# kofinandi/pixel-nerf-yolo

Measured on AMD Instinct MI355X. Metric: rays/sec (whole node), 64 samples/ray, 3-view 128×128 render, higher is better.
Workload: dtype f32 (matrix products on f16x2 split operands, fp32 accumulate)

## Files before the change

### pixel-nerf-yolo_amd/csrc/api.hip

```cpp
#include <algorithm>
#include <cmath>
#include <cstdio>
#include <cstdlib>
#include <cstring>
#include <map>
#include <string>
#include <vector>

#include "api_internal.h"

namespace pny {

static thread_local std::string g_err;
void set_error(const std::string& msg) { g_err = msg; }
int hip_fail(hipError_t e, const char* what) {
    g_err = std::string("HIP error: ") + hipGetErrorString(e) + " in " + what;
    return PNY_ERR_HIP;
}
int fail(int code, const std::string& msg) {
    g_err = msg;
    return code;
}

}
// ... 741 lines not shown
                           const float* focal_dev, const float* c_dev, const float* bboxes_dev,
                           const pny_train_batch_draws* draws, float* rays_dev, float* rgb_gt_dev, int32_t* pix_dev,
                           pny_stream stream) {
    const char* who = "pny_sample_train_batch: ";
    if (!d || !images_dev || !poses_dev || !focal_dev || !rays_dev || !rgb_gt_dev)
        return fail(PNY_ERR_ARG, std::string(who) + "null argument");
    if (d->n_objs < 1 || d->n_views < 1 || d->height < 1 || d->width < 1 || d->n_rays < 1)
        return fail(PNY_ERR_ARG, std::string(who) + "bad shape");
    if ((int64_t)d->n_objs * d->n_rays > INT32_MAX) return fail(PNY_ERR_ARG, std::string(who) + "more than 2^31 - 1 rays");
    if ((int64_t)d->n_views * d->height * d->width > (int64_t)UINT32_MAX)
        return fail(PNY_ERR_ARG, std::string(who) + "NV * H * W must be below 2^32");
    if ((d->focal_rows != 1 && d->focal_rows != d->n_objs) || (d->focal_cols != 1 && d->focal_cols != 2))
        return fail(PNY_ERR_ARG, std::string(who) + "focal must be (1 | SB, 1 | 2)");
    if (c_dev && d->c_rows != 1 && d->c_rows != d->n_objs) return fail(PNY_ERR_ARG, std::string(who) + "c must be (1 | SB, 2)");
    if (draws && (bboxes_dev ? (!draws->image_ids_dev || !draws->u_x_dev || !draws->u_y_dev) : !draws->pix_inds_dev))
        return fail(PNY_ERR_ARG, std::string(who) + (bboxes_dev ? "bbox mode replays image_ids_dev, u_x_dev and u_y_dev"
                                                                : "uniform mode replays pix_inds_dev"));
    if (reinterpret_cast<uintptr_t>(rays_dev) & 15) return fail(PNY_ERR_ARG, std::string(who) + "rays_dev must be 16-byte aligned");
    TrainBatchArgs a;
    a.sb = d->n_objs, a.nv = d->n_views, a.h = d->height, a.w = d->width, a.b = d->n_rays;
    a.znear = d->z_near, a.zfar = d->z_far;
    a.focal_rows = d->focal_rows, a.focal_cols = d->focal_cols, a.c_rows = c_dev ? d->c_rows : 1;
    a.seed = d->seed, a.draw_offset = draws ? 0 : d->draw_offset;
    a.images = images_dev, a.poses = poses_dev, a.focal = focal_dev, a.c = c_dev, a.bboxes = bboxes_dev;
    a.pix_inds = draws && !bboxes_dev ? draws->pix_inds_dev : nullptr;
    a.image_ids = draws && bboxes_dev ? draws->image_ids_dev : nullptr;
    a.u_x = draws && bboxes_dev ? draws->u_x_dev : nullptr;
    a.u_y = draws && bboxes_dev ? draws->u_y_dev : nullptr;
    a.rays = rays_dev, a.rgb = rgb_gt_dev, a.pix = pix_dev;
    launch_train_batch(a, (hipStream_t)stream);
    PNY_HIP(hipGetLastError());
    return PNY_OK;
}

int pny_yolo_train_batch(const pny_yolo_batch_desc* d, const float* poses_host, const int64_t* view_ids_host, const float focal[2],
                         const float c[2], const float* const* targets_dev, float* rays_dev, float* targets_out_dev,
                         int64_t* offsets_host, pny_stream stream) {
    const std::string who = "pny_yolo_train_batch: ";
    if (!d || !offsets_host) return fail(PNY_ERR_ARG, who + "null argument");
    const bool query = !rays_dev && !targets_out_dev;
    if (!query && (!poses_host || !view_ids_host || !focal || !c || !targets_dev || !rays_dev || !targets_out_dev))
        return fail(PNY_ERR_ARG, who + "null argument");
    if (d->n_scales < 1 || d->n_scales > PNY_YOLO_BATCH_MAX_SCALES) return fail(PNY_ERR_ARG, who + "n_scales must be 1 .. 4");
    if (d->n_views < 1 || d->n_views > PNY_YOLO_BATCH_MAX_VIEWS)
        return fail(PNY_ERR_ARG, who + "n_views must be 1 .. 16 (one launch carries at most 16 selected cameras)");
    if (d->n_views_all < 1 || d->height < 1 || d->width < 1) return fail(PNY_ERR_ARG, who + "bad shape");
    if (d->n_anchors < 1 || d->n_anchors > 64) return fail(PNY_ERR_ARG, who + "bad shape: n_anchors must be 1 .. 64");
    if ((reinterpret_cast<uintptr_t>(rays_dev) & 15) || (reinterpret_cast<uintptr_t>(targets_out_dev) & 3))
        return fail(PNY_ERR_ARG, who + "rays_dev must be 16-byte aligned (targets_out_dev 4-byte)");
    YoloBatchArgs a;
    memset(&a, 0, sizeof(a));
    a.n_scales = d->n_scales, a.row = d->n_anchors * 6;
    a.znear = d->z_near, a.zfar = d->z_far;
    a.rays = rays_dev, a.targets_out = targets_out_dev;
    if (!query && (focal[0] == 0.f || focal[1] == 0.f)) return fail(PNY_ERR_ARG, who + "zero focal length");
    for (int s = 0; s < d->n_scales; ++s) {
        const int cell = d->cell_sizes[s];
        if (cell < 1 || cell > d->height || cell > d->width)
            return fail(PNY_ERR_ARG, who + "every cell size must be 1 .. min(height, width)");
        a.hs[s] = d->height / cell, a.ws[s] = d->width / cell;
        a.off[s + 1] = a.off[s] + (long long)d->n_views * a.hs[s] * a.ws[s];
        if ((long long)d->n_views_all * a.hs[s] * a.ws[s] > INT32_MAX) return fail(PNY_ERR_ARG, who + "more than 2^31 - 1 cells in a grid");
        if (query) continue;
        if (!targets_dev[s] || (reinterpret_cast<uintptr_t>(targets_dev[s]) & 3)) return fail(PNY_ERR_ARG, who + "null or unaligned target grid");
        a.targets[s] = targets_dev[s];
        const float fx = focal[0] / (float)cell, fy = focal[1] / (float)cell, cx = c[0] / (float)cell, cy = c[1] / (float)cell;
        a.kinv[s][0] = (float)(1.0 / fx);
        a.kinv[s][1] = (float)(1.0 / fy);
        a.kinv[s][2] = (float)(-(double)cx / fx);
        a.kinv[s][3] = (float)(-(double)cy / fy);
    }
    if (a.off[d->n_scales] * a.row > INT32_MAX) return fail(PNY_ERR_ARG, who + "more than 2^31 - 1 target values");
    if (query) {
        for (int s = 0; s <= d->n_scales; ++s) offsets_host[s] = a.off[s];
        return PNY_OK;
    }
    for (int i = 0; i < d->n_views; ++i) {
        const int64_t v = view_ids_host[i];
        if (v < 0 || v >= d->n_views_all) return fail(PNY_ERR_ARG, who + "view id outside [0, n_views_all)");
        double inv[16];
        if (!invert4(poses_host + 16 * v, inv)) return fail(PNY_ERR_ARG, who + "singular extrinsic matrix");
        for (int r = 0; r < 3; ++r) {
            for (int q = 0; q < 3; ++q) a.pose[i][3 * r + q] = (float)inv[4 * r + q];
            a.pose[i][9 + r] = (float)inv[4 * r + 3];
        }
        a.view_id[i] = (int)v;
    }
    for (int s = 0; s <= d->n_scales; ++s) offsets_host[s] = a.off[s];
    launch_yolo_train_batch(a, (hipStream_t)stream);
    PNY_HIP(hipGetLastError());
    return PNY_OK;
}

}

namespace pny {
static unsigned range_bits(const pny_model* m) {
    return m->range_flag ? __atomic_load_n(m->range_flag, __ATOMIC_RELAXED) : 0u;
}
int check_ready(pny_scene* s, const char* who) {
    if (!s) return fail(PNY_ERR_ARG, std::string(who) + ": null scene");
    if (!s->m->finalized) return fail(PNY_ERR_STATE, std::string(who) + ": weights not finalized (pny_model_finalize)");
    const unsigned bits = s->precision == PNY_PRECISION_F32 ? 0u : range_bits(s->m);
    if (bits) {
        if (bits & PNY_RANGE_WEIGHT) s->m->f16_weights_ok = false;
        return fail(PNY_ERR_RANGE, std::string(who) + ": an earlier f16 (F16X2 / F16) launch left the f16 range (" +
                                       std::string(bits & PNY_RANGE_ACTIVATION ? "activation " : "") +
                                       std::string(bits & PNY_RANGE_GRADIENT ? "gradient " : "") +
                                       std::string(bits & PNY_RANGE_WEIGHT ? "weight " : "") +
                                       "beyond +-65504 or not finite): its results are invalid.  Clear with pny_model_range_status(m, 0, 1), pin "
                                       "pny_scene_set_precision(s, PNY_PRECISION_F32) and repeat the call");
    }
    if (!s->have_latent) return fail(PNY_ERR_STATE, std::string(who) + ": scene has no latent (pny_scene_encode / pny_scene_set_latent)");
    if (!s->have_cams) return fail(PNY_ERR_STATE, std::string(who) + ": scene has no cameras (pny_scene_set_cameras)");
    if (s->cam_ns != s->ns) return fail(PNY_ERR_STATE, std::string(who) + ": camera count != latent view count");
    if (s->n_objs > 1 && s->ns % s->n_objs)
        return fail(PNY_ERR_STATE, std::string(who) + ": grouped scene: the view count is not a multiple of the object count");
    if (obj_views(s) > 1 && s->m->desc.combine_layer >= s->m->desc.n_blocks)
        return fail(PNY_ERR_ARG, std::string(who) + ": multi-view scene needs combine_layer < n_blocks");
    return 0;
}

int view_blocks(const pny_model_desc& d) { return d.combine_layer < d.n_blocks ? d.combine_layer : d.n_blocks; }
}

namespace pny {
double mlp_flops_per_point(const pny_model_desc& d, int ns, MlpPass pass) {
    const int nvb = view_blocks(d);
    const double per_view = (pass == PASS_CHAIN ? 0.0 : (double)d_in(d) * HID) +
                            (pass == PASS_FORWARD ? (double)nvb * d.d_latent * HID : 0.0) + 2.0 * nvb * HID * HID;
    const double post = 2.0 * (d.n_blocks - nvb) * HID * HID + (double)HID * d.d_out;
    const double once = pass == PASS_FORWARD_VIEW_MEAN ? (double)(ns - 1) * HID * HID : 0.0;
    return 2.0 * (ns * per_view + post - once);
}
}

enum MlpKernel { K_F32_8x64 = MLP_8x64, K_F32_16x64 = MLP_16x64, K_F32_8x32 = MLP_8x32, K_H2, K_H2S, K_H1 };
struct MlpRoute {
    MlpKernel kernel;
    Prec prec;
    bool stash;
    bool projected;
    int tile;
    int grid_cap;
};

static bool f16_default(const pny_scene* s) {
    const pny_model* m = s->m;
    return s->precision != PNY_PRECISION_F32 && m->f16_weights_ok && mlp_h2_supports(m->desc.n_blocks, m->desc.combine_layer);
}

static bool wants_projection(const pny_scene* s, long long n_points, bool force) {
    if (!s->m->has_zproj) return false;
    if ((long long)s->hl * s->wl * view_blocks(s->m->desc) * HID >= (1ll << 31)) return false;
    if (force) return true;
    if (s->zp_mode == PNY_PROJECTION_OFF) return false;
    return s->zp_mode != PNY_PROJECTION_AUTO || f16_default(s) || n_points >= 2ll * s->hl * s->wl;
}

static MlpRoute route_mlp(const pny_scene* s, long long n_points, bool stash) {
    const pny_model_desc& d = s->m->desc;
    const int prec = s->precision;
    const bool can_f16 = prec != PNY_PRECISION_F32 && (s->m->f16_weights_ok || prec == PNY_PRECISION_F16X2) &&
                         mlp_h2_supports(d.n_blocks, d.combine_layer) && (!stash || s->L % 128 == 0);
    MlpRoute r;
    r.stash = stash;
    r.projected = stash ? can_f16 && wants_projection(s, n_points, true) : wants_projection(s, n_points, false);
    const bool f16 = r.projected && can_f16;
    const bool h1 = f16 && (prec == PNY_PRECISION_F16_TRAIN || (prec == PNY_PRECISION_F16 && !stash));
    bool h2s = f16 && !h1 && !stash && n_points <= 32ll * mlp_max_grid(MLP_8x64);
    if (f16 && !h1 && !stash)
        if (const char* e = getenv("PNYOLO_H2_SPLIT")) h2s = atoi(e) != 0;
    const int shape = (f16 || stash) ? MLP_8x64 : mlp_pick_variant(n_points);
    r.kernel = h1 ? K_H1 : h2s ? K_H2S : f16 ? K_H2 : MlpKernel(shape);
    r.prec = h1 ? PREC_H1 : f16 ? PREC_H2 : PREC_F32;
    r.tile = h2s ? 32 : mlp_tile_samples(shape);
    r.grid_cap = h2s ? 2 * mlp_max_grid(MLP_8x64) : mlp_max_grid(shape);
    if (!stash)
        if (const char* e = getenv("PNYOLO_GRID")) {
            const int g = atoi(e);
            if (g > 0 && g < r.grid_cap) r.grid_cap = g;
        }
    return r;
}

namespace pny {
static int project_latent(const pny_scene* s, int which, float* out, hipStream_t st, int* route) {
    const pny_model* m = s->m;
    if (!m->desc.has_fine) which = 0;
    const long long npix = (long long)s->ns * s->hl * s->wl;
    if (!run_pixel_linear(m->zproj[which], s->latent.f(), npix, out, st, f16_default(s), route))
        return fail(PNY_ERR_HIP, "latent projection launch failed");
    return 0;
}

int ensure_projection(pny_scene* s, int which, long long n_points, hipStream_t st, const float** zp, bool force) {
    *zp = nullptr;
    const pny_model* m = s->m;
    if (!wants_projection(s, n_points, force)) return 0;
    const int nvb = view_blocks(m->desc);
    if (s->zp_generation != m->generation) {
        s->zp_valid[0] = s->zp_valid[1] = false;
        s->zp_generation = m->generation;
    }
    if (!m->desc.has_fine) which = 0;
    if (!s->zp_valid[which]) {
        const long long npix = (long long)s->ns * s->hl * s->wl;
        int rc;
        if ((rc = s->zp[which].reserve((size_t)npix * nvb * HID * sizeof(float)))) return rc;
        if ((rc = project_latent(s, which, s->zp[which].f(), st, nullptr))) return rc;
        s->zp_valid[which] = true;
    }
    *zp = s->zp[which].f();
    return 0;
}
}

namespace pny {
int fill_mlp_args(pny_scene* s, int mode, const float* xyz, const float* dirs, const float* rays, const float* z, int K,
                  long long n_points, int coarse, float* out, MlpArgs* pa) {
    const pny_model_desc& d = s->m->desc;
    MlpArgs& a = *pa;
    memset(&a, 0, sizeof(a));
    const bool fine_w = !(coarse || !d.has_fine || !s->m->use_fine);
    a.w = fine_w ? s->m->fine : s->m->coarse;
    a.n_blocks = d.n_blocks;
    use_images(a, f16_images(s->m, fine_w, false));
    a.range_flag = s->m->range_flag;
    a.latent = s->latent.f();
    a.zp = nullptr;
    a.zp_stride = view_blocks(d) * HID;
    a.tap_stride = s->L;
    memcpy(a.cams, s->cams, sizeof(Cam) * (size_t)s->ns);
    a.xyz = xyz;
    a.dirs = dirs;
    a.rays = rays;
    a.z = z;
    a.out = out;
    a.n_points = n_points;
    a.K = K;
    a.mode = mode;
    a.NS = obj_views(s);
    a.obj_pts = 0;
    if (s->n_objs > 1) {
        if (n_points % s->n_objs || (n_points / s->n_objs) % 64)
            return fail(PNY_ERR_ARG, "grouped scene: every object's share of the samples must be the same multiple of 64");
        a.obj_pts = n_points / s->n_objs;
    }
    a.L = s->L;
    a.Hl = s->hl;
    a.Wl = s->wl;
    a.combine_layer = d.combine_layer;
    a.d_out = d.d_out;
    a.yolo = d.yolo;
    a.num_freqs = d.num_freqs;
    a.freq_factor = d.freq_factor;
    const float lsx = (float)s->wl / ((float)s->wl - 1.0f) * 2.0f;
    const float lsy = (float)s->hl / ((float)s->hl - 1.0f) * 2.0f;
    a.sx = lsx / (float)s->width;
    a.sy = lsy / (float)s->height;
    const long long tiles = (n_points + 63) / 64;
    if (tiles > 0x7fffffffll) return fail(PNY_ERR_ARG, "too many points for one launch");
    a.n_tiles = (int)tiles;
    a.idx32 = (tiles * 64) < 0xffffffffll;
    if (mode == 1 && (reinterpret_cast<uintptr_t>(rays) & 15)) return fail(PNY_ERR_ARG, "rays must be 16-byte aligned");
    int rc;
    if ((rc = s->scratch.reserve(mlp_scratch_floats() * sizeof(float)))) return rc;
    a.scratch = s->scratch.f();
    return 0;
}
}

static int run_mlp(pny_scene* s, int mode, const float* xyz, const float* dirs, const float* rays, const float* z,
                   int K, long long n_points, int coarse, float* out, hipStream_t st, int stash_pass = -1) {
    if (n_points == 0) return 0;
    pny_model* m = s->m;
    const pny_model_desc& d = m->desc;
    MlpArgs a;
    int rc;
    if ((rc = fill_mlp_args(s, mode, xyz, dirs, rays, z, K, n_points, coarse, out, &a))) return rc;
    const bool fine_w = !(coarse || !d.has_fine || !m->use_fine);
    const int which = fine_w ? 1 : 0;
    bool room = false;
    if (stash_pass >= 0) {
        s->stashed[stash_pass].valid = false;
        room = m->defer && obj_views(s) == m->defer_ns && m->defer_used[which] + a.n_tiles <= m->defer_cap[which];
    }
    const MlpRoute r = route_mlp(s, n_points, room);
    if (r.stash) {
        pny_scene::StashedPass& sp = s->stashed[stash_pass];
        a.lay = stash_layout(d, obj_views(s), s->L);
        a.stash_x = a.lay.x_record(m->dx_stash[which].f(), m->defer_used[which]);
        sp.valid = true;
        sp.epoch = m->defer_epoch;
        sp.which = which;
        sp.tile0 = m->defer_used[which];
        sp.tiles = a.n_tiles;
        sp.n_points = n_points;
        m->defer_used[which] += a.n_tiles;
    }
    if (r.projected) {
        if ((rc = ensure_projection(s, which, n_points, st, &a.zp, r.stash))) return rc;
        a.tap_stride = a.zp_stride;
    }
    if (r.kernel == K_H1) {
        if ((rc = want_h1_images(m, s->precision == PNY_PRECISION_F16_TRAIN))) return rc;
        use_images(a, f16_images(m, fine_w, true));
// ... 274 lines not shown
```

### pixel-nerf-yolo_amd/csrc/mlp_h2.hip

```cpp
#include <cstdlib>
#include <cstring>
#include <cstdio>
#include <vector>

#include "mlp_bwd_core.h"
#include "mlp_h2_core.h"

#if PNY_H2_PLANES == 1
#define PNY_H2_KERNEL pny_mlp_h1_kernel
#elif defined(PNY_H2_SPLIT)
#define PNY_H2_KERNEL pny_mlp_h2s_kernel
#else
#define PNY_H2_KERNEL pny_mlp_h2_kernel
#endif

namespace pny {

#ifdef PNY_H2_STAMP
enum { HS_TOTAL = 0, HS_GEMM, HS_GATHER_WAIT, HS_GATHER, HS_EPI_WAIT, HS_EPI, HS_PROLOGUE, HS_LINOUT, HS_SLAB, HS_REAL, HS_N };
__device__ unsigned long long* g_h2_stamp_buf;
__device__ __forceinline__ unsigned long long h2now() {
    unsigned long long t;
    __builtin_amdgcn_sched_barrier(0);
    asm volatile("s_memtime %0\n\ts_waitcnt lgkmcnt(0)" : "=s"(t)::"memory");
// ... 57 lines not shown
            }
            __builtin_amdgcn_sched_barrier(0);
#pragma unroll
            for (int q = 0; q < 4; ++q) {
                char* s0 = base + (4 * nt + q) * (2 * ROW_BYTES) + 32 * mt * 16;
                float x0 = acc[nt][mt][4 * q + 0] + b[q].x, x1 = acc[nt][mt][4 * q + 1] + b[q].y;
                float x2 = acc[nt][mt][4 * q + 2] + b[q].z, x3 = acc[nt][mt][4 * q + 3] + b[q].w;
                if (ADDZ) {
                    x0 += za[q].x;
                    x1 += za[q].y;
                    x2 += zb[q].x;
                    x3 += zb[q].y;
                }
                acc[nt][mt][4 * q + 0] = x0;
                acc[nt][mt][4 * q + 1] = x1;
                acc[nt][mt][4 * q + 2] = x2;
                acc[nt][mt][4 * q + 3] = x3;
                const float r0 = relu1(x0), r1 = relu1(x1), r2 = relu1(x2), r3 = relu1(x3);
                if constexpr (STASH) stash_store(stash, stash_lane, stash_off + (unsigned)(((8 * nt + 2 * q) * TM + 32 * mt) * 16), r0, r1, r2, r3);
                h2put_planes(s0, r0, r1, r2, r3, rmax);
            }
        }
    }
    range_check(rmax, range_flag);
}

struct SlabRef {
    __amdgpu_buffer_rsrc_t rsrc;
    unsigned lane_off;
};
__device__ __forceinline__ void h2slab_store(const f32x16 (&h)[h2::NT][h2::MT], const SlabRef& sl) {
    using namespace h2;
#pragma unroll
    for (int nt = 0; nt < NT; ++nt)
#pragma unroll
        for (int mt = 0; mt < MT; ++mt)
#pragma unroll
            for (int q = 0; q < 4; ++q) {
                const f32x4 v = {h[nt][mt][4 * q + 0], h[nt][mt][4 * q + 1], h[nt][mt][4 * q + 2], h[nt][mt][4 * q + 3]};
                __builtin_amdgcn_raw_buffer_store_b128(__builtin_bit_cast(u32x4, v), sl.rsrc,
                                                       sl.lane_off + (unsigned)(((nt * MT + mt) * 4 + q) * 64 * 16), 0, 2);
            }
}
__device__ __forceinline__ void h2slab_load(f32x16 (&t)[h2::NT][h2::MT], const SlabRef& sl) {
    using namespace h2;
#pragma unroll
    for (int nt = 0; nt < NT; ++nt)
#pragma unroll
        for (int mt = 0; mt < MT; ++mt)
#pragma unroll
            for (int q = 0; q < 4; ++q) {
                const u32x4 u = __builtin_amdgcn_raw_buffer_load_b128(sl.rsrc, sl.lane_off, (unsigned)(((nt * MT + mt) * 4 + q) * 64 * 16), 2);
                const f32x4 v = __builtin_bit_cast(f32x4, u);
                t[nt][mt][4 * q + 0] = v.x;
                t[nt][mt][4 * q + 1] = v.y;
                t[nt][mt][4 * q + 2] = v.z;
                t[nt][mt][4 * q + 3] = v.w;
            }
}

#ifndef PNY_H2_SLAB_DEPTH
#define PNY_H2_SLAB_DEPTH 4
#endif
struct SlabPipe {
    static constexpr int SD = PNY_H2_SLAB_DEPTH;
    static_assert(SD >= 2, "slab pipeline");
    f32x4 buf[SD][4];
};
__device__ __forceinline__ void h2slab_issue(SlabPipe& sp, int p, const SlabRef& sh, const SlabRef& sr) {
    const SlabRef& s = (p & 1) ? sh : sr;
#pragma unroll
    for (int q = 0; q < 4; ++q)
        sp.buf[p % SlabPipe::SD][q] =
            __builtin_bit_cast(f32x4, __builtin_amdgcn_raw_buffer_load_b128(s.rsrc, s.lane_off, (unsigned)(((p >> 1) * 4 + q) * 64 * 16), 2));
}
__device__ __forceinline__ void h2view_sum(f32x16 (&net)[h2::NT][h2::MT], f32x16 (&h)[h2::NT][h2::MT], const float* bias, const SlabRef& sh,
                                           const SlabRef& sr, bool add, bool store, int wave, int lane) {
    using namespace h2;
    SlabPipe sp;
    const float* bl = bias + 32 * NT * wave + 4 * (lane >> 5);
    constexpr int NP = 2 * NT * MT, SD = SlabPipe::SD;
    if (add) {
#pragma unroll
        for (int p = 0; p + 1 < SD; ++p) h2slab_issue(sp, p, sh, sr);
    }
#pragma unroll
    for (int p = 0; p < NP; ++p) {
        const int nt = (p >> 1) / MT, mt = (p >> 1) % MT;
        if (add) {
            if (p + SD - 1 < NP) h2slab_issue(sp, p + SD - 1, sh, sr);
            __builtin_amdgcn_sched_barrier(0);
        }
        f32x16& t = (p & 1) ? h[nt][mt] : net[nt][mt];
#pragma unroll
        for (int q = 0; q < 4; ++q) {
            if (!(p & 1)) {
                const float4 b = *reinterpret_cast<const float4*>(bl + 32 * nt + 8 * q);
                t[4 * q + 0] = relu1(t[4 * q + 0] + b.x);
                t[4 * q + 1] = relu1(t[4 * q + 1] + b.y);
                t[4 * q + 2] = relu1(t[4 * q + 2] + b.z);
                t[4 * q + 3] = relu1(t[4 * q + 3] + b.w);
            }
            if (add) {
#pragma unroll
                for (int i = 0; i < 4; ++i) t[4 * q + i] = t[4 * q + i] + sp.buf[p % SD][q][i];
            }
            if (store) {
                const SlabRef& s = (p & 1) ? sh : sr;
                const f32x4 v = {t[4 * q + 0], t[4 * q + 1], t[4 * q + 2], t[4 * q + 3]};
                __builtin_amdgcn_raw_buffer_store_b128(__builtin_bit_cast(u32x4, v), s.rsrc, s.lane_off + (unsigned)(((p >> 1) * 4 + q) * 64 * 16), 0, 2);
            }
        }
        if (add) __builtin_amdgcn_sched_barrier(0);
    }
}

__device__ __forceinline__ void h2mean_planes(const f32x16 (&net)[h2::NT][h2::MT], f32x16 (&h)[h2::NT][h2::MT], float rns, char* planes, int wave,
                                              int lane, unsigned* range_flag) {
    using namespace h2;
    float rmax = 0.f;
    char* base = planes + (4 * NT * wave) * (2 * ROW_BYTES) + (lane & 31) * 16 + 8 * (lane >> 5);
#pragma unroll
    for (int nt = 0; nt < NT; ++nt)
#pragma unroll
        for (int mt = 0; mt < MT; ++mt)
#pragma unroll
            for (int q = 0; q < 4; ++q) {
                char* s0 = base + (4 * nt + q) * (2 * ROW_BYTES) + 32 * mt * 16;
                const float r0 = net[nt][mt][4 * q + 0] * rns, r1 = net[nt][mt][4 * q + 1] * rns;
                const float r2 = net[nt][mt][4 * q + 2] * rns, r3 = net[nt][mt][4 * q + 3] * rns;
                h2put_planes(s0, r0, r1, r2, r3, rmax);
#pragma unroll
                for (int i = 0; i < 4; ++i) h[nt][mt][4 * q + i] = h[nt][mt][4 * q + i] * rns;
            }
    range_check(rmax, range_flag);
}

template <int B>
__device__ __forceinline__ void h2gather_commit(const GatherTaps<h2::C, 2>& g, char* planes, int chunk, int wave, int lane) {
    using namespace h2;
    constexpr int NMB = GatherTaps<C>::NMB, QSTEP = GatherTaps<C>::QSTEP;
    const int m = (wave % NMB) * 8 + (lane & 7);
    char* base = planes + (16 * chunk + (lane >> 4)) * (2 * ROW_BYTES) + m * 16 + 8 * ((lane >> 3) & 1);
#pragma unroll
    for (int i = 0; i < GatherTaps<C>::QPW; ++i) {
        const int qb = wave / NMB + i * QSTEP;
        const float4 r = tap_blend(g.x[B][i], g.w);
        char* s0 = base + (4 * qb) * (2 * ROW_BYTES);
        *reinterpret_cast<float2*>(s0) = make_float2(r.x, r.y);
        *reinterpret_cast<float2*>(s0 + ROW_BYTES) = make_float2(r.z, r.w);
    }
}

template <bool STASH>
__device__ __forceinline__ void h2prologue(const MlpArgs& a, int v, long long tile, char* planes, float4* tap_tab, int tid, unsigned* range_flag,
                                           __amdgpu_buffer_rsrc_t stash = __amdgpu_buffer_rsrc_t(), unsigned stash_xin = 0, float4* tap_raw = nullptr) {
    using namespace h2;
    constexpr int NPART = THREADS / TM;
    const int m = tid % TM, part = tid / TM;
    long long s = tile * TM + m;
    if (s >= a.n_points) s = a.n_points - 1;
    float p[3], d[3];
    load_point(a, s, p, d);
    const Cam cam = a.cams[tile_view_base(a, tile * TM) + v];
    float xr[3], xc[3], vd[3];
    camera_point(cam, p, d, xr, xc, vd);
    float rmax = 0.f;
    for (int g = part; g < D_IN_PAD / 4; g += NPART) {
        const float e0 = input_entry(4 * g + 0, xr, vd, a.freq_factor, a.num_freqs), e1 = input_entry(4 * g + 1, xr, vd, a.freq_factor, a.num_freqs);
        const float e2 = input_entry(4 * g + 2, xr, vd, a.freq_factor, a.num_freqs), e3 = input_entry(4 * g + 3, xr, vd, a.freq_factor, a.num_freqs);
        if constexpr (STASH) stash_store(stash, (unsigned)((g * TM + m) * 16), stash_xin, e0, e1, e2, e3);
        h2put_planes<true>(planes + (g >> 1) * (2 * ROW_BYTES) + m * 16 + 8 * (g & 1), e0, e1, e2, e3, rmax);
    }
    range_check(rmax, range_flag);
    if (part == NPART - 1) {
        int pix[4], offs[4];
        float wgt[4];
        pixel_taps(a, cam, xc, 1, pix, wgt);
#pragma unroll
        for (int k = 0; k < 4; ++k) offs[k] = pix[k] * a.tap_stride;
        tap_record(tap_tab, m, offs, wgt);
        if constexpr (STASH) {
#pragma unroll
            for (int k = 0; k < 4; ++k) offs[k] = pix[k] * a.L;
            tap_record(tap_raw, m, offs, wgt);
        }
    }
}

template <bool STASH>
__global__ __launch_bounds__(h2::THREADS, 2) void PNY_H2_KERNEL(const MlpArgs a) {
    using namespace h2;
    extern __shared__ __attribute__((aligned(16))) char smem_raw[];
    char* planes = smem_raw;
    float4* tap_tab = reinterpret_cast<float4*>(smem_raw + ACT_BYTES);
    float* bias_tab = reinterpret_cast<float*>(smem_raw + ACT_BYTES + TAP_BYTES);
    float4* tap_raw = reinterpret_cast<float4*>(smem_raw + lds_bytes(a.n_blocks));
    const int tid = threadIdx.x, lane = tid & 63, wave = __builtin_amdgcn_readfirstlane(tid >> 6);
    const SlabRef slab = {__builtin_amdgcn_make_buffer_rsrc(a.scratch + (size_t)blockIdx.x * (TM * HID), 0, TM * HID * 4, 0x00020000),
                          (unsigned)((wave * (NT * MT * 16 * 64) + 4 * lane) * 4)};
#if defined(PNY_H2_PER_VIEW_FC1) || PNY_H2_PLANES == 1
    constexpr bool VIEW_MEAN = false;
#else
    constexpr bool VIEW_MEAN = !STASH;
#endif
    const SlabRef slab_r = {__builtin_amdgcn_make_buffer_rsrc(a.scratch + ((size_t)gridDim.x + blockIdx.x) * (TM * HID), 0, TM * HID * 4, 0x00020000),
                            slab.lane_off};
    const int nb = a.n_blocks;
    const int nvb = a.combine_layer < nb ? a.combine_layer : nb;
    const WStream ws = wstream(a, lane);
    const H2Seg s_in = h2seg(ws, a.h2_in, D_IN_PAD / 16, wave);
    auto fc0seg = [&](int b) { return h2seg(ws, a.h2_fc0[b], HID / 16, wave); };
    auto fc1seg = [&](int b) { return h2seg(ws, a.h2_fc1[b], HID / 16, wave); };
    auto entry_bias = [&](int b) -> const float* {
        if constexpr (LDS_BIAS) return bias_tab + (b == 0 ? 0 : 2 * b) * HID;
        return b == 0 ? a.w.b_in : a.w.b_fc1[b - 1];
    };
    auto fc0_bias = [&](int b) -> const float* {
        if constexpr (LDS_BIAS) return bias_tab + (1 + 2 * b) * HID;
        return a.w.b_fc0[b];
    };
    H2Ring ring;
    h2ring_fill(ring, ws, s_in);
#ifdef PNY_H2_STAMP
    unsigned long long hs_acc[HS_N], hs_t_ = 0;
    for (int i = 0; i < HS_N; ++i) hs_acc[i] = 0;
    const unsigned long long hs_start = h2now();
    const unsigned long long hs_real0 = __builtin_amdgcn_s_memrealtime();
#endif
    if constexpr (LDS_BIAS) {
        for (int i = tid; i < (1 + 2 * nb) * HID; i += THREADS) {
            const int vec = i / HID, f = i % HID;
            const float* src = vec == 0 ? a.w.b_in : ((vec & 1) ? a.w.b_fc0[(vec - 1) >> 1] : a.w.b_fc1[(vec - 2) >> 1]);
            bias_tab[i] = src[f];
        }
    }

    const TileWalk tw = tile_walk(a.n_tiles);
    for (long long tile = tw.first; tile < tw.last; tile += tw.step) {
        f32x16 h[NT][MT];
        f32x16 net[NT][MT];
        GatherTaps<C, 2> g;
        __amdgpu_buffer_rsrc_t xr = __amdgpu_buffer_rsrc_t();
        if constexpr (STASH)
            xr = stash_rsrc(a.lay.x_record(a.stash_x, tile), a.lay.x_tile);
        auto block_tail = [&](int blk, const H2Seg& after, bool slab_in, int next_c0, unsigned stash_net) {
            HS_T0();
            h2zero<NT, MT>(net);
            __syncthreads();
            HS_LAP(HS_EPI_WAIT);
            h2gemm(net, ring, ws, fc0seg(blk), fc1seg(blk), planes, lane);
            HS_LAP(HS_GEMM);
            __syncthreads();
            HS_LAP(HS_EPI_WAIT);
            h2epilogue<false, STASH>(net, fc0_bias(blk), planes, wave, lane, a.range_flag, xr, stash_net);
            if (!VIEW_MEAN && slab_in) {
                h2slab_load(net, slab);
                HS_LAP(HS_EPI);
                __syncthreads();
                HS_LAP(HS_EPI_WAIT);
                h2gemm(h, ring, ws, fc1seg(blk), after, planes, lane);
                HS_LAP(HS_GEMM);
#pragma unroll
                for (int nt = 0; nt < NT; ++nt)
#pragma unroll
                    for (int mt = 0; mt < MT; ++mt)
#pragma unroll
                        for (int r = 0; r < 16; ++r) h[nt][mt][r] = net[nt][mt][r] + h[nt][mt][r];
            } else if (next_c0 >= 0) {
                HS_LAP(HS_EPI);
                __syncthreads();
                HS_LAP(HS_EPI_WAIT);
                h2gemm(h, ring, ws, fc1seg(blk), after, planes, lane, [&]() { gather_issue<C, 0>(g, next_c0, wave); });
                HS_LAP(HS_GEMM);
            } else {
                HS_LAP(HS_EPI);
                __syncthreads();
                HS_LAP(HS_EPI_WAIT);
                h2gemm(h, ring, ws, fc1seg(blk), after, planes, lane);
                HS_LAP(HS_GEMM);
            }
        };
        for (int v = 0; v < a.NS; ++v) {
            const int vb = tile_view_base(a, tile * TM);
            const H2Seg after_view = v + 1 < a.NS ? s_in : (nvb < nb ? fc0seg(nvb) : s_in);
            const unsigned x_view = STASH ? stash_bytes((unsigned)v * (unsigned)a.lay.x_view) : 0u;
            auto act_slot = [&](int i) { return x_view + stash_bytes((unsigned)a.lay.o_act + (unsigned)i * (unsigned)STASH_SLOT); };
            HS_T0();
            __syncthreads();
            h2prologue<STASH>(a, v, tile, planes, tap_tab, tid, a.range_flag, xr, x_view + stash_bytes((unsigned)a.lay.o_in), tap_raw);
            h2zero<NT, MT>(h);
            __syncthreads();
            if constexpr (STASH) {
                const unsigned xz = x_view + stash_bytes((unsigned)a.lay.o_z);
                gather_setup<C>(g, a.latent + (size_t)(vb + v) * a.Hl * a.Wl * a.L, tap_raw, wave, lane);
                const int nch = a.L / GCH;
                const unsigned zlane = (unsigned)(((lane >> 3) * TM + (wave % 8) * 8 + (lane & 7)) * 16);
                auto put = [&](const float4(&x)[4][4], int c) {
#pragma unroll
                    for (int i = 0; i < 4; ++i) {
                        const float4 r = tap_blend(x[i], g.w);
                        stash_store(xr, zlane, xz + (unsigned)((32 * c + 8 * i) * TM * 16), r.x, r.y, r.z, r.w);
                    }
                };
                gather_issue<C, 0>(g, 0, wave);
                for (int c = 0; c < nch; c += 2) {
                    if (c + 1 < nch) gather_issue<C, 1>(g, (c + 1) * GCH, wave);
                    __builtin_amdgcn_sched_barrier(0);
                    put(g.x[0], c);
                    if (c + 2 < nch) gather_issue<C, 0>(g, (c + 2) * GCH, wave);
                    __builtin_amdgcn_sched_barrier(0);
                    if (c + 1 < nch) put(g.x[1], c + 1);
                }
            }
            gather_setup<C>(g, a.zp + (size_t)(vb + v) * a.Hl * a.Wl * a.zp_stride, tap_tab, wave, lane);
            gather_issue<C, 0>(g, 0, wave);
            HS_LAP(HS_PROLOGUE);
            h2gemm(h, ring, ws, s_in, fc0seg(0), planes, lane);
            HS_LAP(HS_GEMM);
            auto block_entry = [&](int blk) {
                const int cb = blk * HID;
                HS_LAP(HS_GATHER);
                __syncthreads();
                HS_LAP(HS_GATHER_WAIT);
                gather_issue<C, 1>(g, cb + GCH, wave);
                __builtin_amdgcn_sched_barrier(0);
                h2gather_commit<0>(g, planes, 0, wave, lane);
                gather_issue<C, 0>(g, cb + 2 * GCH, wave);
                __builtin_amdgcn_sched_barrier(0);
                h2gather_commit<1>(g, planes, 1, wave, lane);
                gather_issue<C, 1>(g, cb + 3 * GCH, wave);
                __builtin_amdgcn_sched_barrier(0);
                h2gather_commit<0>(g, planes, 2, wave, lane);
                h2gather_commit<1>(g, planes, 3, wave, lane);
                HS_LAP(HS_GATHER);
                __syncthreads();
                HS_LAP(HS_GATHER_WAIT);
                h2epilogue<true, STASH>(h, entry_bias(blk), planes, wave, lane, a.range_flag, xr, act_slot(2 * blk));
                HS_LAP(HS_EPI);
            };
            auto view_block = [&](int blk, const H2Seg& after, bool slab_in, int next_c0) {
                block_entry(blk);
                block_tail(blk, after, slab_in, next_c0, act_slot(2 * blk + 1));
            };
            auto mean_tail = [&](int blk) {
                const bool last = v + 1 == a.NS;
                HS_T0();
                h2zero<NT, MT>(net);
                __syncthreads();
                HS_LAP(HS_EPI_WAIT);
                h2gemm(net, ring, ws, fc0seg(blk), last ? fc1seg(blk) : s_in, planes, lane);
                HS_LAP(HS_GEMM);
                h2view_sum(net, h, fc0_bias(blk), slab, slab_r, v > 0, !last, wave, lane);
                if (!last) {
                    HS_LAP(HS_SLAB);
                    return;
                }
                HS_LAP(v > 0 ? HS_SLAB : HS_EPI);
                __syncthreads();
                HS_LAP(HS_EPI_WAIT);
                h2mean_planes(net, h, 1.0f / (float)a.NS, planes, wave, lane, a.range_flag);
                HS_LAP(HS_EPI);
                __syncthreads();
                HS_LAP(HS_EPI_WAIT);
                h2gemm(h, ring, ws, fc1seg(blk), after_view, planes, lane);
                HS_LAP(HS_GEMM);
            };
#if defined(PNY_H2_NOPREFETCH)
            for (int blk = 0; blk + 1 < nvb; ++blk) {
                view_block(blk, fc0seg(blk + 1), false, -1);
                gather_issue<C, 0>(g, (blk + 1) * HID, wave);
            }
#else
            for (int blk = 0; blk + 1 < nvb; ++blk) view_block(blk, fc0seg(blk + 1), false, (blk + 1) * HID);
#endif
            if constexpr (VIEW_MEAN) {
                block_entry(nvb - 1);
                mean_tail(nvb - 1);
            } else {
                view_block(nvb - 1, after_view, v > 0, -1);
            }
            if (!VIEW_MEAN && a.NS > 1) {
                HS_T0();
                if (v + 1 < a.NS) {
                    h2slab_store(h, slab);
                } else {
                    const float rns = 1.0f / (float)a.NS;
#pragma unroll
                    for (int nt = 0; nt < NT; ++nt)
#pragma unroll
                        for (int mt = 0; mt < MT; ++mt)
#pragma unroll
                            for (int r = 0; r < 16; ++r) h[nt][mt][r] = h[nt][mt][r] * rns;
                }
                HS_LAP(HS_SLAB);
            }
        }
        auto post_slot = [&](int i) { return stash_bytes((unsigned)a.lay.x_post + (unsigned)i * (unsigned)STASH_SLOT); };
        for (int blk = nvb; blk < nb; ++blk) {
            HS_T0();
            __syncthreads();
            HS_LAP(HS_EPI_WAIT);
            h2epilogue<false, STASH>(h, entry_bias(blk), planes, wave, lane, a.range_flag, xr, post_slot(2 * (blk - nvb)));
            HS_LAP(HS_EPI);
            block_tail(blk, blk + 1 < nb ? fc0seg(blk + 1) : s_in, false, -1, post_slot(2 * (blk - nvb) + 1));
        }
        HS_T0();
        __syncthreads();
        h2epilogue<false, STASH>(h, entry_bias(nb), planes, wave, lane, a.range_flag, xr, post_slot(2 * (nb - nvb)));
        __syncthreads();
        for (int idx = tid; idx < a.d_out * TM; idx += THREADS) {
            const int o = idx / TM, m = idx % TM;
            const float4* wrow = reinterpret_cast<const float4*>(a.w.w_out + (size_t)o * HID);
            float sum = 0.f;
#pragma unroll 4
            for (int kg = 0; kg < HID / 8; ++kg) {
                const h8 x0 = *reinterpret_cast<const h8*>(planes + kg * (2 * ROW_BYTES) + m * 16);
                const float4 wa = wrow[2 * kg], wb = wrow[2 * kg + 1];
                if constexpr (PL == 1) {
                    sum += (float)x0[0] * wa.x;
                    sum += (float)x0[1] * wa.y;
                    sum += (float)x0[2] * wa.z;
                    sum += (float)x0[3] * wa.w;
                    sum += (float)x0[4] * wb.x;
                    sum += (float)x0[5] * wb.y;
                    sum += (float)x0[6] * wb.z;
                    sum += (float)x0[7] * wb.w;
                } else {
                    const h8 x1 = *reinterpret_cast<const h8*>(planes + kg * (2 * ROW_BYTES) + ROW_BYTES + m * 16);
                    sum += ((float)x0[0] + (float)x1[0]) * wa.x;
                    sum += ((float)x0[1] + (float)x1[1]) * wa.y;
                    sum += ((float)x0[2] + (float)x1[2]) * wa.z;
                    sum += ((float)x0[3] + (float)x1[3]) * wa.w;
                    sum += ((float)x0[4] + (float)x1[4]) * wb.x;
                    sum += ((float)x0[5] + (float)x1[5]) * wb.y;
                    sum += ((float)x0[6] + (float)x1[6]) * wb.z;
                    sum += ((float)x0[7] + (float)x1[7]) * wb.w;
                }
            }
            sum = output_head(sum + a.w.b_out[o], o, a.yolo);
            const long long s = tile * TM + m;
            if (s < a.n_points) a.out[s * a.d_out + o] = sum;
        }
        HS_LAP(HS_LINOUT);
    }
#ifdef PNY_H2_STAMP
    hs_acc[HS_TOTAL] = h2now() - hs_start;
    hs_acc[HS_REAL] = __builtin_amdgcn_s_memrealtime() - hs_real0;
    if (lane == 0)
        for (int i = 0; i < HS_N; ++i) g_h2_stamp_buf[((size_t)blockIdx.x * (THREADS / 64) + wave) * HS_N + i] = hs_acc[i];
#endif
}

#if !defined(PNY_H2_SPLIT) && PNY_H2_PLANES == 2
bool mlp_h2_supports(int n_blocks, int combine_layer) { return n_blocks <= h2::MAX_NB && combine_layer >= 1; }
#endif

template <bool STASH>
static void launch_mlp_h2_t(const MlpArgs& a, int grid, hipStream_t st) {
    const int extra = STASH ? h2::TAP_BYTES : 0;
    static LdsLimit lds;
    (void)lds.raise(h2::lds_bytes(h2::MAX_NB) + extra, PNY_H2_KERNEL<STASH>);
#ifdef PNY_H2_STAMP
    static unsigned long long* dbuf = nullptr;
    constexpr int NWV = h2::THREADS / 64;
    const size_t nst = (size_t)grid * NWV * HS_N;
    if (!dbuf) {
        (void)hipMalloc((void**)&dbuf, (size_t)1024 * 8 * HS_N * sizeof(unsigned long long));
        (void)hipMemcpyToSymbol(HIP_SYMBOL(g_h2_stamp_buf), &dbuf, sizeof(dbuf));
    }
    (void)hipMemsetAsync(dbuf, 0, nst * sizeof(unsigned long long), st);
#endif
    hipLaunchKernelGGL(PNY_H2_KERNEL<STASH>, dim3(grid), dim3(h2::THREADS), h2::lds_bytes(a.n_blocks) + extra, st, a);
#ifdef PNY_H2_STAMP
    {
        std::vector<unsigned long long> hst(nst);
        (void)hipStreamSynchronize(st);
        (void)hipMemcpy(hst.data(), dbuf, nst * sizeof(unsigned long long), hipMemcpyDeviceToHost);
        double sum[HS_N] = {0};
        for (size_t i = 0; i < nst; ++i) sum[i % HS_N] += (double)hst[i];
        static const char* names[HS_N] = {"total", "gemm", "gather-barrier-wait", "gather", "epilogue-barrier-wait", "epilogue", "prologue", "lin_out", "slab", "realtime"};
        fprintf(stderr, "[h2 stamp%s, %d x %d] tiles=%d grid=%d:", STASH ? ", stash" : "", h2::NT, h2::MT, a.n_tiles, grid);
        for (int i = 0; i < HS_N; ++i) fprintf(stderr, " %s=%.1f%%", names[i], 100.0 * sum[i] / sum[0]);
        fprintf(stderr, " (mean wave cycles %.4g; in-kernel clock %.3f GHz = wave cycles / s_memrealtime ticks x 100 MHz)\n",
                sum[0] / ((double)grid * NWV), sum[0] / sum[HS_REAL] * 0.1);
    }
#endif
}

#if PNY_H2_PLANES == 1 && defined(PNY_H1_STASH)
void launch_mlp_h1_stash(const MlpArgs& a, int grid, hipStream_t st) { launch_mlp_h2_t<true>(a, grid, st); }
#elif PNY_H2_PLANES == 1
void launch_mlp_h1(const MlpArgs& a, int grid, hipStream_t st) { launch_mlp_h2_t<false>(a, grid, st); }
#elif defined(PNY_H2_SPLIT)
void launch_mlp_h2s(const MlpArgs& a, int grid, hipStream_t st) { launch_mlp_h2_t<false>(a, grid, st); }
#else
void launch_mlp_h2(const MlpArgs& a, int grid, hipStream_t st) { launch_mlp_h2_t<false>(a, grid, st); }
void launch_mlp_h2_stash(const MlpArgs& a, int grid, hipStream_t st) { launch_mlp_h2_t<true>(a, grid, st); }
#endif

}
```

Measured before the change: 215,100.

## Gather z-projection per wave and fuse into block-entry epilogue without block barriers

```diff
diff --git a/pixel-nerf-yolo_amd/csrc/api.hip b/pixel-nerf-yolo_amd/csrc/api.hip
--- a/pixel-nerf-yolo_amd/csrc/api.hip
+++ b/pixel-nerf-yolo_amd/csrc/api.hip
@@ -917,7 +917,7 @@
 
 static bool wants_projection(const pny_scene* s, long long n_points, bool force) {
     if (!s->m->has_zproj) return false;
-    if ((long long)s->hl * s->wl * view_blocks(s->m->desc) * HID >= (1ll << 31)) return false;
+    if ((long long)s->hl * s->wl * view_blocks(s->m->desc) * HID >= (1ll << 30)) return false;
     if (force) return true;
     if (s->zp_mode == PNY_PROJECTION_OFF) return false;
     return s->zp_mode != PNY_PROJECTION_AUTO || f16_default(s) || n_points >= 2ll * s->hl * s->wl;
diff --git a/pixel-nerf-yolo_amd/csrc/mlp_h2.hip b/pixel-nerf-yolo_amd/csrc/mlp_h2.hip
--- a/pixel-nerf-yolo_amd/csrc/mlp_h2.hip
+++ b/pixel-nerf-yolo_amd/csrc/mlp_h2.hip
@@ -233,6 +233,88 @@
     }
 }
 
+struct WaveGather {
+    f32x4 x[2][4][4];
+};
+template <int B, int T>
+__device__ __forceinline__ void h2wave_issue(WaveGather& wg, __amdgpu_buffer_rsrc_t zr, const float4* tap_tab, unsigned c0, int lane) {
+    using namespace h2;
+    constexpr int nt = T / MT, mt = T % MT;
+    asm volatile("" : "+v"(lane));
+    const float4* tt = tap_tab + 2 * (32 * mt + (lane >> 3));
+    const unsigned ql = 16u * (unsigned)(lane & 7);
+#pragma unroll
+    for (int pass = 0; pass < 4; ++pass) {
+        const float4 o = tt[16 * pass];
+        const unsigned off[4] = {(unsigned)__float_as_int(o.x), (unsigned)__float_as_int(o.y), (unsigned)__float_as_int(o.z), (unsigned)__float_as_int(o.w)};
+#pragma unroll
+        for (int k = 0; k < 4; ++k)
+            wg.x[B][pass][k] = __builtin_bit_cast(f32x4, __builtin_amdgcn_raw_buffer_load_b128(zr, off[k] * 4u + ql, c0 + 128u * nt, 0));
+    }
+}
+template <int B, int T>
+__device__ __forceinline__ void h2wave_commit(const WaveGather& wg, f32x16 (&acc)[h2::NT][h2::MT], const float4* tap_tab, const float* bias,
+                                              char* planes, int wave, int lane, float& rmax) {
+    using namespace h2;
+    constexpr int nt = T / MT, mt = T % MT;
+    const int jq = lane & 7, sl = lane >> 3, m0 = lane & 31, hh = lane >> 5;
+    char* tb = planes + (4 * NT * wave + 4 * nt) * (2 * ROW_BYTES) + 32 * mt * 16;
+    char* wr = tb + jq * ROW_BYTES + 16 * (sl ^ jq);
+    const float4* tw = tap_tab + 2 * (32 * mt + sl) + 1;
+#pragma unroll
+    for (int pass = 0; pass < 4; ++pass) {
+        const float4 w4 = tw[16 * pass];
+        const float w[4] = {w4.x, w4.y, w4.z, w4.w};
+        float4 x[4];
+#pragma unroll
+        for (int k = 0; k < 4; ++k) x[k] = make_float4(wg.x[B][pass][k][0], wg.x[B][pass][k][1], wg.x[B][pass][k][2], wg.x[B][pass][k][3]);
+        *reinterpret_cast<float4*>(wr + 128 * pass) = tap_blend(x, w);
+    }
+    __builtin_amdgcn_fence(__ATOMIC_RELEASE, "wavefront");
+    __builtin_amdgcn_wave_barrier();
+    __builtin_amdgcn_fence(__ATOMIC_ACQUIRE, "wavefront");
+    const float* bl = bias + 32 * NT * wave + 32 * nt + 4 * hh;
+    auto rd_b = [&](int q) { return *reinterpret_cast<const float4*>(bl + 8 * q); };
+    auto rd_z = [&](int q) { return *reinterpret_cast<const float4*>(tb + (2 * q + hh) * ROW_BYTES + 16 * (m0 ^ (2 * q + hh))); };
+    float4 b = rd_b(0), z = rd_z(0);
+#pragma unroll
+    for (int q = 0; q < 4; ++q) {
+        const float4 bq = b, zq = z;
+        if (q + 1 < 4) b = rd_b(q + 1), z = rd_z(q + 1);
+        __builtin_amdgcn_fence(__ATOMIC_ACQ_REL, "wavefront");
+        char* s0 = tb + q * (2 * ROW_BYTES) + m0 * 16 + 8 * hh;
+        float x0 = acc[nt][mt][4 * q + 0] + bq.x, x1 = acc[nt][mt][4 * q + 1] + bq.y;
+        float x2 = acc[nt][mt][4 * q + 2] + bq.z, x3 = acc[nt][mt][4 * q + 3] + bq.w;
+        x0 += zq.x;
+        x1 += zq.y;
+        x2 += zq.z;
+        x3 += zq.w;
+        acc[nt][mt][4 * q + 0] = x0;
+        acc[nt][mt][4 * q + 1] = x1;
+        acc[nt][mt][4 * q + 2] = x2;
+        acc[nt][mt][4 * q + 3] = x3;
+        const float r0 = relu1(x0), r1 = relu1(x1), r2 = relu1(x2), r3 = relu1(x3);
+        h2put_planes(s0, r0, r1, r2, r3, rmax);
+    }
+}
+__device__ __forceinline__ void h2wave_entry(WaveGather& wg, f32x16 (&acc)[h2::NT][h2::MT], __amdgpu_buffer_rsrc_t zr, const float4* tap_tab, unsigned c0,
+                                             const float* bias, char* planes, int wave, int lane, unsigned* range_flag) {
+    static_assert(h2::NT * h2::MT == 4, "four sub-chunks");
+    asm volatile("" : "+v"(lane));
+    float rmax = 0.f;
+    h2wave_issue<1, 1>(wg, zr, tap_tab, c0, lane);
+    __builtin_amdgcn_sched_barrier(0);
+    h2wave_commit<0, 0>(wg, acc, tap_tab, bias, planes, wave, lane, rmax);
+    h2wave_issue<0, 2>(wg, zr, tap_tab, c0, lane);
+    __builtin_amdgcn_sched_barrier(0);
+    h2wave_commit<1, 1>(wg, acc, tap_tab, bias, planes, wave, lane, rmax);
+    h2wave_issue<1, 3>(wg, zr, tap_tab, c0, lane);
+    __builtin_amdgcn_sched_barrier(0);
+    h2wave_commit<0, 2>(wg, acc, tap_tab, bias, planes, wave, lane, rmax);
+    h2wave_commit<1, 3>(wg, acc, tap_tab, bias, planes, wave, lane, rmax);
+    range_check(rmax, range_flag);
+}
+
 template <bool STASH>
 __device__ __forceinline__ void h2prologue(const MlpArgs& a, int v, long long tile, char* planes, float4* tap_tab, int tid, unsigned* range_flag,
                                            __amdgpu_buffer_rsrc_t stash = __amdgpu_buffer_rsrc_t(), unsigned stash_xin = 0, float4* tap_raw = nullptr) {
@@ -285,6 +367,7 @@
 #else
     constexpr bool VIEW_MEAN = !STASH;
 #endif
+    constexpr bool WAVE_ENTRY = !STASH;
     const SlabRef slab_r = {__builtin_amdgcn_make_buffer_rsrc(a.scratch + ((size_t)gridDim.x + blockIdx.x) * (TM * HID), 0, TM * HID * 4, 0x00020000),
                             slab.lane_off};
     const int nb = a.n_blocks;
@@ -322,6 +405,15 @@
         f32x16 h[NT][MT];
         f32x16 net[NT][MT];
         GatherTaps<C, 2> g;
+        WaveGather wg;
+        __amdgpu_buffer_rsrc_t zr = __amdgpu_buffer_rsrc_t();
+        const unsigned wave_c0 = (unsigned)(32 * NT * wave) * 4u;
+        auto prefetch = [&](int c0) {
+            if constexpr (WAVE_ENTRY)
+                h2wave_issue<0, 0>(wg, zr, tap_tab, (unsigned)c0 * 4u + wave_c0, lane);
+            else
+                gather_issue<C, 0>(g, c0, wave);
+        };
         __amdgpu_buffer_rsrc_t xr = __amdgpu_buffer_rsrc_t();
         if constexpr (STASH)
             xr = stash_rsrc(a.lay.x_record(a.stash_x, tile), a.lay.x_tile);
@@ -352,7 +444,7 @@
                 HS_LAP(HS_EPI);
                 __syncthreads();
                 HS_LAP(HS_EPI_WAIT);
-                h2gemm(h, ring, ws, fc1seg(blk), after, planes, lane, [&]() { gather_issue<C, 0>(g, next_c0, wave); });
+                h2gemm(h, ring, ws, fc1seg(blk), after, planes, lane, [&]() { prefetch(next_c0); });
                 HS_LAP(HS_GEMM);
             } else {
                 HS_LAP(HS_EPI);
@@ -394,8 +486,13 @@
                     if (c + 1 < nch) put(g.x[1], c + 1);
                 }
             }
-            gather_setup<C>(g, a.zp + (size_t)(vb + v) * a.Hl * a.Wl * a.zp_stride, tap_tab, wave, lane);
-            gather_issue<C, 0>(g, 0, wave);
+            if constexpr (WAVE_ENTRY) {
+                const size_t zfloats = (size_t)a.Hl * a.Wl * a.zp_stride;
+                zr = __builtin_amdgcn_make_buffer_rsrc(const_cast<float*>(a.zp) + (size_t)(vb + v) * zfloats, 0, (int)(unsigned)(zfloats * 4), 0x00020000);
+            } else {
+                gather_setup<C>(g, a.zp + (size_t)(vb + v) * a.Hl * a.Wl * a.zp_stride, tap_tab, wave, lane);
+            }
+            prefetch(0);
             HS_LAP(HS_PROLOGUE);
             h2gemm(h, ring, ws, s_in, fc0seg(0), planes, lane);
             HS_LAP(HS_GEMM);
@@ -404,6 +501,11 @@
                 HS_LAP(HS_GATHER);
                 __syncthreads();
                 HS_LAP(HS_GATHER_WAIT);
+                if constexpr (WAVE_ENTRY) {
+                    h2wave_entry(wg, h, zr, tap_tab, (unsigned)cb * 4u + wave_c0, entry_bias(blk), planes, wave, lane, a.range_flag);
+                    HS_LAP(HS_GATHER);
+                    return;
+                }
                 gather_issue<C, 1>(g, cb + GCH, wave);
                 __builtin_amdgcn_sched_barrier(0);
                 h2gather_commit<0>(g, planes, 0, wave, lane);
@@ -450,7 +552,7 @@
 #if defined(PNY_H2_NOPREFETCH)
             for (int blk = 0; blk + 1 < nvb; ++blk) {
                 view_block(blk, fc0seg(blk + 1), false, -1);
-                gather_issue<C, 0>(g, (blk + 1) * HID, wave);
+                prefetch((blk + 1) * HID);
             }
 #else
             for (int blk = 0; blk + 1 < nvb; ++blk) view_block(blk, fc0seg(blk + 1), false, (blk + 1) * HID);
```

After: 228,100 (median of 6 runs). 1.06x the previous value.
